# dobraczka/kiez

Hardware: AMD Instinct MI355X
Metric: source queries/sec (fit+kneighbors) + recall@k vs reference, 1/2/4/8 GPU (higher is better)
Workload: dtype f16

## Files before the change

kiez_amd/csrc/kz_common.h:

```cpp
#pragma once
#include <hip/hip_runtime.h>

#include <cstdarg>
#include <cstdint>
#include <cstdio>
#include <cstring>
#include <memory>

#include "../../include/kiez_amd.h"
#include "kz_pool_buf.h"

#define KZ_TILE 128
#define KZ_KSLICE 16
#define KZ_LIVE_MAX 1024
#define KZ_POOL_SLOTS 256

constexpr int KZ_K_LDS_PAD = 0;
constexpr int KZ_K_LONG_K = 1;
constexpr int KZ_K_FIN_WIDE = 1;
constexpr int KZ_K_RANGE_BOOT = 1;
constexpr double KZ_K_NESTED_MIN_MS = 2.0;
constexpr int KZ_K_DUAL_SHORT_DIV = 5;
constexpr int KZ_K_DUAL_SHORT_KP = 16;
constexpr int KZ_K_MIN_SPLITS = 1;
// ... 12 lines not shown
    hipStream_t stream;
    bool own_stream;
    hipEvent_t ev[12];
    int stream2_busy;
    hipStream_t stream2;
    double eps_scale;
    int force_splits;
    int chunk_rows;
    int precision;
    int dual_stride;
    int esc_bf;
    int short_ord_min_tiles;
    int short_ord;
    int dual_short_main;
    int dual_rev_long;
    int dual_short_extra;
    int dual_short_min_tiles;
    int dual_sample_short;
    int dual_overlap;
    double dual_max_gb;
    int dual_force;
    int h_q64;
    int fin_fast_div;
    double probe_min_pairs;
    int list_floor;
    int tier_probe;
    int dual_nested;
    int esc_ladder;
    int exact_rows;
    int abl;
    double floor_margin;
    int dual_rank;
    int spec_rows;
    int wide_lists;
    int wide_sel;
    void* scratch;
    size_t scratch_bytes;
    float* floor_buf;
    size_t floor_bytes;
    int* d_counters;
    int* h_counters;
    int n_cus;
    void* h_stage;
    size_t h_stage_bytes;
    int h_stage_flip;
    struct { void* ptr; size_t bytes; } pool[KZ_POOL_SLOTS];
// ... 324 lines not shown
```

kiez_amd/csrc/kz_knn.hip:

```cpp
#include <vector>

#include <algorithm>
#include <type_traits>

#include "kz_common.h"
#include "kz_bool.h"
#include "kz_floor.h"

#include "kz_knn_device.h"

template <int KP, int NRES>
__global__ __launch_bounds__(256, 3) void kz_knn_cand_kernel(KnnCandParams p) {
    extern __shared__ __attribute__((aligned(16))) char smem[];
    float* ybuf = reinterpret_cast<float*>(smem);
    const int tid = threadIdx.x;
    const int lane = tid & 63;
    const int wave = tid >> 6;
    const int j = lane & 31;
    const int h = lane >> 5;

    const int4 wd = p.work[blockIdx.x];
    const int qt = wd.x;
    const int t_begin = wd.y;
    const int t_end = wd.z;
// ... 115 lines not shown
            if (NRES == 0 || NS > NRES) {
                int sl = NRES;
                do {
                    const int sln = (sl + 1 == NS) ? NRES : sl + 1;
                    const float4 c0 = qb0, c1 = qb1;
                    slice_step(c0, c1, true, sln);
                } while (++sl < NS);
            }
            __builtin_amdgcn_sched_barrier(0);
            kz_tile_epilogue<KP>(acc, st, tile, tile == t_end - 1, h);
        }
    }
}

#include "kz_knn_bf16.h"


struct KnnFinParams {
    const float* in_key;
    const int* in_idx;
    KzListLayout lay;
    int max_m;
    int fast_div;
    int64_t q_first, q_last;
    int KP;
    int KSEL;
    int64_t list_row0;
    int64_t q_begin;
    int64_t q_count;
    const void* qraw;
    const void* yraw;
    const double* ynorm64;
    const double* qsqn;
    const double* ysqn;
    int64_t n_i;
    int d;
    int metric;
    int k;
    int exclude_self;
    const int64_t* self_ids;
    double gamma;
    const double* ystats;
    int tier_h;
    double eps_mult;
    double gamma_acc;
    const double* q_rowq;
// ... 33 lines not shown
        const int lim = min(n_sorted, k + 1);
        for (int c = 0; c < lim; ++c)
            if ((int64_t)sidx[c] == self_row) {
                self_rank = c;
                break;
            }
    }
    for (int c = lane; c < n_sorted; c += 64) {
        if (c == self_rank) continue;
        const int o = (self_rank >= 0 && c > self_rank) ? c - 1 : c;
        if (o < k) {
            od[o] = kz_output_distance<T>(sval[c], metric, p);
            oi[o] = (int64_t)sidx[c];
        }
    }
}

#ifndef KZ_FIN_ROWS_N
#define KZ_FIN_ROWS_N 1
#endif
#ifndef KZ_FIN_DEPTH
#define KZ_FIN_DEPTH 3
#endif
constexpr int KZ_FIN_ROWS = KZ_FIN_ROWS_N;
constexpr int KZ_FIN_MAXM = 4096;
constexpr int KZ_ESC_SHORT_MAX_ROWS = 2048;
constexpr int KZ_MAX_PIECES = 128;
static int kz_max_pieces(int KP, int halves) {
    const int m = KZ_FIN_MAXM / (halves * KP);
    return m < KZ_MAX_PIECES ? m : KZ_MAX_PIECES;
}

__host__ __device__ __forceinline__ int kz_fin_wave_bytes(int max_m, int KP) {
    return ((max_m * 8 + KP * 28) + 15) & ~15;
}
__host__ __device__ __forceinline__ int kz_fin_wide_wave_bytes(int max_m, int KS) {
    return ((max_m * 8 + KS * 20) + 15) & ~15;
}

template <int E>
__device__ __forceinline__ float kz_full_lists_bound(const float (&key)[E], const bool (&ok)[E], int M, int KP, int lane) {
    float bound = -INFINITY;
#pragma unroll
    for (int i = 0; i < E; ++i) {
        if (64 * i >= M) break;
        int c = ok[i] ? 1 : 0;
// ... 138 lines not shown
#pragma unroll
    for (int v = 0; v < E; ++v) {
        n_valid += __popcll(__ballot(xi[v] >= 0));
        const int lim = min(64, M - 64 * v);
        for (int jj = 0; jj < lim; ++jj) {
            const int oi = __builtin_amdgcn_readlane(xi[v], jj);
            if (oi < 0) continue;
            const float ox = __uint_as_float((unsigned)__builtin_amdgcn_readlane((int)__float_as_uint(x[v]), jj));
#pragma unroll
            for (int u = 0; u < E; ++u)
                if (64 * u < M) rank[u] += (ox > x[u] || (ox == x[u] && oi < xi[u])) ? 1 : 0;
        }
    }
#pragma unroll
    for (int u = 0; u < E; ++u) {
        if (xi[u] >= 0 && rank[u] < KP) {
            ck[rank[u]] = x[u];
            ci[rank[u]] = xi[u];
        }
    }
    return n_valid < KP ? n_valid : KP;
}

template <typename T, int FROWS, int NV = 1>
__device__ __forceinline__ void kz_finalize_query(const KnnFinParams& p, const int64_t q, const int lane, char* wbase) {
    const int KS = p.KSEL > 0 ? p.KSEL : p.KP;
    double* cv = reinterpret_cast<double*>(wbase);
    double* sv = cv + KS;
    float* ekey = reinterpret_cast<float*>(sv + KS);
    int* eidx = reinterpret_cast<int*>(ekey + p.max_m);
    float* ck = reinterpret_cast<float*>(eidx + p.max_m);
    int* ci = reinterpret_cast<int*>(ck + KS);
    int* si = ci + KS;
    const int KP = p.KP;
    const int k_eff = p.k + (p.exclude_self ? 1 : 0);
    const int64_t qrow = p.row_map ? (int64_t)p.row_map[p.q_begin + q] : p.q_begin + q;
    const int64_t qout = p.row_map ? qrow : q;
    const T* qptr = reinterpret_cast<const T*>(p.qraw) + qrow * (int64_t)p.d;
    const double qs = p.qsqn[qrow];

    const int64_t lrow = p.list_row0 + q;
    const int n_pieces = p.lay.pieces[kz_list_region(lrow, p.lay)];
    const int halves = p.lay.halves;
    const int M = n_pieces * halves * KP;
    if (p.lay.contig) {
        const int64_t l0 = kz_list_contig_off(lrow, p.lay, KP, 0);
        for (int e = lane; e < M; e += 64) {
// ... 146 lines not shown
                } else if (c < V) {
                    left_max = fmaxf(left_max, ck[c]);
                }
                cnt += (int)__popcll(mask);
            }
#pragma unroll
            for (int off = 32; off >= 1; off >>= 1) left_max = fmaxf(left_max, __shfl_xor(left_max, off, 64));
            Vr = cnt;
            ck = ekey;
            ci = eidx;
            kz_wave_sync();
        }
    } else if (V > k_eff && eps_q < INFINITY) {
        const double thr = (double)ck[k_eff - 1] * key_scale - 2.0 * eps_q;
        int cnt = 0;
        for (int c = lane; c < V; c += 64) cnt += ((double)ck[c] * key_scale >= thr) ? 1 : 0;
#pragma unroll
        for (int off = 32; off >= 1; off >>= 1) cnt += __shfl_xor(cnt, off, 64);
        Vr = cnt < k_eff ? k_eff : cnt;
    }

    const T* yraw = reinterpret_cast<const T*>(p.yraw);
    const bool vec = kz_row_vec_ok(qptr, p.d) && kz_row_vec_ok(yraw, p.d);
#ifdef KZ_NO_FIN_PIPE
    if (false) {
#else
    if (sizeof(T) == 4 && vec && p.d <= 256 * NV && Vr > 0) {
#endif
        const int k0 = 4 * lane;
        bool act[NV];
        int k0r[NV];
        double qk[4 * NV];
#pragma unroll
        for (int c = 0; c < NV; ++c) {
            act[c] = k0 + 256 * c < p.d;
            k0r[c] = act[c] ? k0 + 256 * c : 0;
            double t[4] = {0.0, 0.0, 0.0, 0.0};
            if (act[c]) {
                kz_row4(qptr, k0r[c], p.d, true, t);
                if (p.metric == KZ_COSINE) {
#pragma unroll
                    for (int e = 0; e < 4; ++e) t[e] = t[e] / qs;
                }
            }
#pragma unroll
            for (int e = 0; e < 4; ++e) qk[4 * c + e] = t[e];
// ... 171 lines not shown
            certified = V >= k_eff && (double)bound * key_scale + eps_q < exact_key(sv[k_eff - 1]);
    }
    if (Vr < V && !((double)(unsorted ? left_max : ck[Vr]) * key_scale + eps_q < exact_key(sv[k_eff - 1]))) certified = false;
    if (bound_violated) certified = false;
    if (!certified) {
        if (lane == 0) {
            const int pos = atomicAdd(p.fail_count, 1);
            p.fail_list[pos] = (int)qout;
            if (p.fail_tau) p.fail_tau[pos] = Vr >= k_eff ? sv[k_eff - 1] : (double)INFINITY;
        }
        return;
    }
    kz_emit_sorted<T>(sv, si, Vr, p.k, p.exclude_self, p.self_ids ? p.self_ids[q] : qrow, p.metric,
                      p.out_dist + qout * (int64_t)p.k, p.out_ind + qout * (int64_t)p.k, lane);
}

constexpr int KZ_FIN_QPB = 4;
#ifndef KZ_FIN_WAVES_2
#define KZ_FIN_WAVES_2 5
#endif
#ifndef KZ_FIN_WAVES
#define KZ_FIN_WAVES 7
#endif
template <typename T, int FROWS, int MINW, int NV = 1>
__global__ __launch_bounds__(256, MINW) void kz_knn_finalize_kernel(KnnFinParams p) {
    extern __shared__ __attribute__((aligned(16))) char fsm[];
    const int lane = threadIdx.x & 63;
    const int wave = __builtin_amdgcn_readfirstlane(threadIdx.x >> 6);
    char* wbase = fsm + (size_t)wave * kz_fin_wave_bytes(p.max_m, p.KSEL > 0 ? p.KSEL : p.KP);
    for (int rep = 0; rep < KZ_FIN_QPB / 4; ++rep) {
        const int64_t q = p.q_first + (int64_t)blockIdx.x * KZ_FIN_QPB + rep * 4 + wave;
        if (q >= p.q_last) break;
        kz_finalize_query<T, FROWS, NV>(p, q, lane, wbase);
        kz_wave_sync();
    }
}

#include "kz_knn_fin_wide.h"

__device__ __forceinline__ bool kz_spec_row_live(const int* __restrict__ dyn_n, int b, int cap) {
    const int n = *dyn_n;
    return n <= cap && b < n;
}

template <typename T>
__global__ __launch_bounds__(256) void kz_exact_dist_kernel(const int* __restrict__ fail_list, int batch0, int64_t q_begin,
                                                            const T* __restrict__ qraw, const T* __restrict__ yraw,
                                                            const double* __restrict__ qsqn, const double* __restrict__ ysqn,
                                                            int64_t n_i, int d, int metric, double p, double* __restrict__ vals,
                                                            const int* __restrict__ dyn_n = nullptr) {
    const int lane = threadIdx.x & 63;
    const int wave = threadIdx.x >> 6;
    const int b = blockIdx.y;
    if (dyn_n && !kz_spec_row_live(dyn_n, b, (int)gridDim.y)) return;
    const int64_t qrow = q_begin + fail_list[batch0 + b];
    for (int64_t i = (int64_t)blockIdx.x * 4 + wave; i < n_i; i += (int64_t)gridDim.x * 4) {
// ... 834 lines not shown
        while (rg + 1 < lay.n_regions && lay.pieces[rg + 1] == lay.pieces[rg]) ++rg;
        const int64_t hi = (int64_t)lay.qt_end[rg] * KZ_TILE - fp.list_row0;
        Group g = {lo < 0 ? 0 : lo, hi > q_count ? q_count : hi, lay.pieces[rg] * lay.halves * KP};
        if (g.hi > g.lo) groups[n_groups++] = g;
    }
    const hipStream_t main_stream = ctx->stream;
    const bool fork = n_groups >= 2 && ctx->stream2 && ctx->stream2 != main_stream && !ctx->stream2_busy;
    int big = 0;
    for (int g = 1; g < n_groups; ++g)
        if (groups[g].hi - groups[g].lo > groups[big].hi - groups[big].lo) big = g;
    if (fork) {
        KZ_HIP(hipEventRecord(ctx->ev[7], main_stream));
        KZ_HIP(hipStreamWaitEvent(ctx->stream2, ctx->ev[7], 0));
    }
    for (int pass = 0; pass < 2; ++pass) {
        for (int g = 0; g < n_groups; ++g) {
            const bool side = fork && g != big;
            if (fork ? (side != (pass == 0)) : pass == 1) continue;
            const hipStream_t st = side ? ctx->stream2 : main_stream;
            fp.q_first = groups[g].lo;
            fp.q_last = groups[g].hi;
            fp.max_m = groups[g].max_m;
            fp.fast_div = ctx->fin_fast_div;
            const int fin_blocks = (int)((fp.q_last - fp.q_first + KZ_FIN_QPB - 1) / KZ_FIN_QPB);
            size_t fin_lds = (size_t)4 * kz_fin_wave_bytes(fp.max_m, fp.KSEL > 0 ? fp.KSEL : KP);
            const bool wide = (fp.KSEL > 0 ? fp.KSEL : KP) > 160;
            const bool rows_vec = fp.d <= 256 && (fp.d & 3) == 0 && (((uintptr_t)fp.qraw | (uintptr_t)fp.yraw) & 15u) == 0;
            const bool wide2 = (wide || (KZ_K_FIN_WIDE >= 2 && fp.KSEL > 0)) && dtype == KZ_F32 && fp.tier_h && !fp.excl_floor && KZ_K_FIN_WIDE && rows_vec;
            const bool two_chunks = !wide && !wide2 && dtype == KZ_F32 && fp.d > 256 && fp.d <= 512 && (fp.d & 3) == 0 &&
                                    (((uintptr_t)fp.qraw | (uintptr_t)fp.yraw) & 15u) == 0;
            const void* fk = two_chunks ? (const void*)kz_knn_finalize_kernel<float, KZ_FIN_ROWS, KZ_FIN_WAVES_2, 2> : dtype == KZ_F32 ? (wide2 ? (const void*)kz_knn_finalize_wide_kernel<float, 4> : (wide ? (const void*)kz_knn_finalize_kernel<float, 8, 2> : (const void*)kz_knn_finalize_kernel<float, KZ_FIN_ROWS, KZ_FIN_WAVES>))
                                             : (wide ? (const void*)kz_knn_finalize_kernel<double, 4, 2> : (const void*)kz_knn_finalize_kernel<double, KZ_FIN_ROWS, KZ_FIN_WAVES>);
            if (wide2) fin_lds = (size_t)4 * kz_fin_wide_wave_bytes(fp.max_m, fp.KSEL);
            if (fin_lds > 65536) KZ_HIP(hipFuncSetAttribute(fk, hipFuncAttributeMaxDynamicSharedMemorySize, (int)fin_lds));
            if (wide2)
                hipLaunchKernelGGL((kz_knn_finalize_wide_kernel<float, 4>), dim3(fin_blocks), dim3(256), fin_lds, st, fp);
            else if (dtype == KZ_F32 && wide)
                hipLaunchKernelGGL((kz_knn_finalize_kernel<float, 8, 2>), dim3(fin_blocks), dim3(256), fin_lds, st, fp);
            else if (dtype == KZ_F32 && two_chunks)
                hipLaunchKernelGGL((kz_knn_finalize_kernel<float, KZ_FIN_ROWS, KZ_FIN_WAVES_2, 2>), dim3(fin_blocks), dim3(256), fin_lds, st, fp);
            else if (dtype == KZ_F32)
                hipLaunchKernelGGL((kz_knn_finalize_kernel<float, KZ_FIN_ROWS, KZ_FIN_WAVES>), dim3(fin_blocks), dim3(256), fin_lds, st, fp);
            else if (wide)
                hipLaunchKernelGGL((kz_knn_finalize_kernel<double, 4, 2>), dim3(fin_blocks), dim3(256), fin_lds, st, fp);
            else
                hipLaunchKernelGGL((kz_knn_finalize_kernel<double, KZ_FIN_ROWS, KZ_FIN_WAVES>), dim3(fin_blocks), dim3(256), fin_lds, st, fp);
        }
    }
    KZ_HIP(hipGetLastError());
    if (fork) {
        KZ_HIP(hipEventRecord(ctx->ev[11], ctx->stream2));
        KZ_HIP(hipStreamWaitEvent(main_stream, ctx->ev[11], 0));
    }
    return KZ_OK;
}

struct KzPass {
    KzListLayout lay;
    int W;
    int W0;
    float* out_key;
    int* out_idx;
    int* fail_list;
// ... 1101 lines not shown
```

kiez_amd/csrc/kz_knn_dual.h:

```cpp
#pragma once

constexpr int KZ_EVC = 1;

__global__ __launch_bounds__(256) void kz_dual_theta_kernel(const float* __restrict__ in_key, const int* __restrict__ in_idx,
                                                            KzListLayout lay, int KP, int rank, int64_t n_b, int64_t n_b_pad,
                                                            const float* __restrict__ bias_b, const double* __restrict__ a_hmax,
                                                            const double* __restrict__ b_hmax, const double* __restrict__ hscale,
                                                            float* __restrict__ theta, float* __restrict__ floor_,
                                                            const int* __restrict__ idx_to_row, int sev_cap, int* __restrict__ sev_cnt,
                                                            uint2* __restrict__ sev) {
    const int lane = threadIdx.x & 63;
    const int64_t t = (int64_t)blockIdx.x * 4 + (threadIdx.x >> 6);
    if (t >= n_b_pad) return;
    if (t >= n_b) {
        if (lane == 0) theta[t] = INFINITY;
        return;
    }
    const int M = lay.pieces[kz_list_region(t, lay)] * KP;
    const int64_t l0 = kz_list_contig_off(t, lay, KP, 0);
    float x[4];
    int valid[4];
    unsigned ux[4];
    unsigned all_or = 0u, all_and = 0xffffffffu;
    int nv = 0;
#pragma unroll
    for (int u = 0; u < 4; ++u) {
        const int e = lane + 64 * u;
        x[u] = e < M ? in_key[l0 + e] : -INFINITY;
        valid[u] = e < M && in_idx[l0 + e] >= 0;
        const unsigned b = __float_as_uint(x[u]);
        ux[u] = valid[u] ? (b ^ ((b >> 31) ? 0xffffffffu : 0x80000000u)) : 0u;
        all_or |= ux[u];
        all_and &= valid[u] ? ux[u] : 0xffffffffu;
        nv += valid[u] ? 1 : 0;
    }
#pragma unroll
// ... 28 lines not shown
            }
        }
        int base = 0;
#pragma unroll
        for (int u = 0; u < 4; ++u) {
            const bool evt = valid[u] && x[u] >= tau && tau > -INFINITY;
            const unsigned long long mask = __ballot(evt);
            if (evt) {
                const int pos = base + (int)__builtin_amdgcn_mbcnt_hi((unsigned)(mask >> 32), __builtin_amdgcn_mbcnt_lo((unsigned)mask, 0u));
                if (pos < sev_cap) sev[t * (int64_t)sev_cap + pos] = make_uint2(__float_as_uint(x[u]), (unsigned)idx_to_row[in_idx[l0 + lane + 64 * u]]);
            }
            base += (int)__popcll(mask);
        }
        if (lane == 0) sev_cnt[t] = base;
    }
    if (lane == 0) {
        const double S2 = hscale[0] * hscale[0];
        const double margin = 4.76837158203125e-07 * S2 * (a_hmax[0] * b_hmax[0] + a_hmax[2] + b_hmax[2]);
        const double th = (double)tau + (double)bias_b[t] - margin;
        float tf = (float)th;
        if ((double)tf > th) tf = nextafterf(tf, -INFINITY);
        theta[t] = tf;
        floor_[t] = tau_bound;
    }
}

__global__ __launch_bounds__(256) void kz_dual_sample_kernel(const uint4* __restrict__ packed, const float* __restrict__ bias,
                                                             int nsr, int stride, int s_tiles, int P,
                                                             uint4* __restrict__ s_packed, float* __restrict__ s_bias) {
    const int jp = blockIdx.x;
    const int n_frag = 2 * nsr * KZ_TILE;
    for (int e = threadIdx.x; e < n_frag; e += 256) {
        const int row = e & (KZ_TILE - 1), blk = e >> 7;
        const int64_t j = kz_dealt_row((int64_t)jp * KZ_TILE + row, (int64_t)s_tiles * KZ_TILE, P);
        const int64_t src_tile = (j >> 7) * stride;
        s_packed[(int64_t)jp * n_frag + e] = packed[src_tile * n_frag + blk * KZ_TILE + (j & (KZ_TILE - 1))];
        if (blk == 0) s_bias[(int64_t)jp * KZ_TILE + row] = bias[src_tile * KZ_TILE + (j & (KZ_TILE - 1))];
    }
}

__global__ void kz_dual_interleave_kernel(const int* __restrict__ perm, const float* __restrict__ theta_s, int64_t n, int64_t n_pad,
                                          int P, int* __restrict__ perm_out, float* __restrict__ theta_out) {
    const int64_t rp = (int64_t)blockIdx.x * blockDim.x + threadIdx.x;
    if (rp >= n_pad) return;
    const int64_t tiles = n_pad / KZ_TILE - 1;
    const int64_t jp = rp / KZ_TILE;
// ... 690 lines not shown
            const int KP = KPs3;
            int blocks_per_cu = 1, tpw = 1;
            KZ_DISPATCH_KP(rc, kz_h_occupancy, (n_slices, &blocks_per_cu, &tpw, KZ_K_H_WPS, KZ_K_H_WIDE, KZ_K_LDS_PAD));
            if (rc != KZ_OK) return rc;
            KzPass ps;
            rc = kz_prepare_pass(ctx, (int)s_tiles, (int)s3_tiles, kz_h_slots(n_slices, blocks_per_cu, ctx->n_cus), 256 / KP, KP, KZ_TIER_H, 0, &ps, tpw, force_s3);
            if (rc == KZ_OK) {
                KnnCandParams cp;
                memset(&cp, 0, sizeof(cp));
                cp.qpack = (const float*)q_packed.get();
                cp.ypack = (const float*)nst.s3_packed.get();
                cp.ybias = nst.s3_bias.get();
                cp.work = ps.d_work;
                cp.qt0 = 0;
                cp.n_ytiles = (int)s3_tiles;
                cp.n_qtiles = (int)s_tiles;
                cp.lay = ps.lay;
                cp.kg = b->kg;
                cp.out_key = ps.out_key;
                cp.out_idx = ps.out_idx;
                KZ_DISPATCH_KP(rc, kz_h_launch, (n_slices, ctx, cp, ps.W, KZ_K_H_WPS, KZ_K_H_WIDE));
            }
            if (rc != KZ_OK) return rc;
            hipLaunchKernelGGL(kz_dual_theta_kernel, dim3((unsigned)((s_img_rows + 3) / 4)), dim3(256), 0, ctx->stream, ps.out_key, ps.out_idx,
                               ps.lay, KP, rank3, s_img_rows, s_img_rows, q_bias.get(), ib->d_max, ia->d_max, ia->center->d_scale, nst.theta3.get(), nst.floor3.get(),
                               (const int*)nullptr, 0, (int*)nullptr, (uint2*)nullptr);
            KZ_HIP(hipGetLastError());
        }
        hipLaunchKernelGGL(kz_iota_kernel, dim3((unsigned)((s_img_rows + 255) / 256)), dim3(256), 0, ctx->stream, nst.iota3.get(), (int)s_img_rows);
        KZ_HIP(hipGetLastError());
        rc = kz_sort_pairs_f32_i32(ctx, nst.theta3.get(), nst.theta3_s.get(), nst.iota3.get(), nst.perm3.get(), (int)s_img_rows, 1);
        if (rc == KZ_OK && force_s > 1) {
            const int64_t range_rows = ((s_tiles + force_s - 1) / force_s) * KZ_TILE;
            hipLaunchKernelGGL(kz_dual_rangekey_kernel, dim3((unsigned)((s_img_rows + 255) / 256)), dim3(256), 0, ctx->stream, nst.perm3.get(), s_img_rows, range_rows,
                               nst.theta3.get(), nst.iota3.get());
            if (hipGetLastError() != hipSuccess) rc = KZ_ERR_HIP;
            if (rc == KZ_OK) rc = kz_sort_pairs_f32_i32(ctx, nst.theta3.get(), nst.floor3m.get(), nst.iota3.get(), nst.rm3.get(), (int)s_img_rows, 0);
            if (rc == KZ_OK) {
                hipLaunchKernelGGL(kz_dual_gather2_kernel, dim3((unsigned)((s_img_rows + 255) / 256)), dim3(256), 0, ctx->stream, nst.rm3.get(), nst.perm3.get(), nst.theta3_s.get(),
                                   s_img_rows, nst.iota3.get(), nst.theta3.get());
                if (hipGetLastError() != hipSuccess) rc = KZ_ERR_HIP;
                std::swap(nst.perm3, nst.iota3);
                std::swap(nst.theta3_s, nst.theta3);
            }
        }
        if (rc == KZ_OK) {
            hipLaunchKernelGGL(kz_dual_rows_of_kernel, dim3((unsigned)((s_img_rows + 255) / 256)), dim3(256), 0, ctx->stream, nst.perm3.get(), row_map.get(), s_img_rows, nst.rm3.get());
// ... 23 lines not shown
        dp2.ypack = (const float*)nst.ss_packed.get();
        dp2.ybias = nst.ss_bias.get();
        dp2.perm = nst.rm3.get();
        dp2.theta = nst.theta3_min.get();
        dp2.qnbias = nst.qnb_b.get();
        dp2.log_keys = nst.log3_keys.get();
        dp2.log_meta = nst.log3_meta.get();
        dp2.log_cnt = nst.d_cnt3.get();
        dp2.log_cap = log_cap3;
        dp2.short_pieces = force_s;
        dp2.short_kp = KPs;
        dp2.short_ksel = k;
        dp2.n_ytiles = (int)s_tiles;
        dp2.raw_lists = 1;
        dp2.max_entries = 256;
        hk2.rm3 = nst.rm3.get();
        hk2.sev_cnt = nst.sev_cnt.get();
        hk2.sev = nst.sev.get();
        dp2.post_user = &hk2;
        dp2.post_sweep = +[](void* user) -> int {
            Hook2& h = *(Hook2*)user;
            kz_ctx* ctx = h.ctx;
            const KzDualPass& d2 = *h.dp2;
            hipLaunchKernelGGL(kz_dual_theta_kernel, dim3((unsigned)((h.b_pad + 3) / 4)), dim3(256), 0, ctx->stream, d2.lists_key, d2.lists_idx,
                               d2.lists_lay, d2.lists_KP, h.rank, h.b_n, h.b_pad, h.ib->bias, h.ia->d_max, h.ib->d_max, h.ib->center->d_scale,
                               h.theta, h.floor_, h.rm3, h.sev_cap, h.sev_cnt, h.sev);
            KZ_HIP(hipGetLastError());
            return kz_dual_enqueue_chain(*h.rv3);
        };
        kz_knn_stats st2;
        ctx->stream2_busy = 1;
        rc = kz_knn_impl(ctx, b, 0, b->n, a, k, 0, nullptr, KzResearch(), d_dist_ba, d_ind_ba, &st2, &dp2);
        if (rc != KZ_OK) return rc;
        if (dp2.broken || !dp2.post_called) {
            then = 1;
            return KZ_OK;
        }
        nested_sweep_ms = st2.main_kernel_ms;
    } else {
        hipLaunchKernelGGL(kz_dual_sample_kernel, dim3((unsigned)s_tiles), dim3(256), 0, ctx->stream, (const uint4*)ia->packed, ia->bias,
                           n_slices, stride, (int)s_tiles, force_s > 0 ? force_s : 1, (uint4*)s_packed.get(), s_bias.get());
        KZ_HIP(hipGetLastError());
        const int KP = KPs;
        int blocks_per_cu = 1, tpw = 1;
        KZ_DISPATCH_KP(rc, kz_h_occupancy, (n_slices, &blocks_per_cu, &tpw, KZ_K_H_WPS, KZ_K_H_WIDE, KZ_K_LDS_PAD));
        if (rc != KZ_OK) return rc;
        KzPass ps;
        rc = kz_prepare_pass(ctx, (int)b_tiles, (int)s_tiles, kz_h_slots(n_slices, blocks_per_cu, ctx->n_cus), 256 / KP, KP, KZ_TIER_H, 0, &ps, tpw, force_s);
        if (rc != KZ_OK) return rc;
        KnnCandParams cp;
        memset(&cp, 0, sizeof(cp));
        cp.qpack = (const float*)ib->packed;
        cp.ypack = (const float*)s_packed.get();
        cp.ybias = s_bias.get();
        cp.work = ps.d_work;
        cp.qt0 = 0;
        cp.n_ytiles = (int)s_tiles;
        cp.n_qtiles = (int)b_tiles;
        cp.lay = ps.lay;
        cp.kg = b->kg;
        cp.out_key = ps.out_key;
        cp.out_idx = ps.out_idx;
        KZ_DISPATCH_KP(rc, kz_h_launch, (n_slices, ctx, cp, ps.W, KZ_K_H_WPS, KZ_K_H_WIDE));
        if (rc != KZ_OK) return rc;
        hipLaunchKernelGGL(kz_dual_theta_kernel, dim3((unsigned)((b_pad + 3) / 4)), dim3(256), 0, ctx->stream, ps.out_key, ps.out_idx,
                           ps.lay, KP, rank, b->n, b_pad, ib->bias, ia->d_max, ib->d_max, ib->center->d_scale, theta.get(), floor_.get(),
                           (const int*)nullptr, 0, (int*)nullptr, (uint2*)nullptr);
        KZ_HIP(hipGetLastError());
    }
    hipLaunchKernelGGL(kz_iota_kernel, dim3((unsigned)((b_pad + 255) / 256)), dim3(256), 0, ctx->stream, iota.get(), (int)b_pad);
    hipLaunchKernelGGL(kz_dual_fill_kernel, dim3((unsigned)((b_pad + 255) / 256)), dim3(256), 0, ctx->stream, theta_s.get(), b_pad, INFINITY);
    KZ_HIP(hipGetLastError());
    rc = kz_sort_pairs_f32_i32(ctx, theta.get(), theta_s.get(), iota.get(), perm.get(), (int)b->n, 1);
    if (rc != KZ_OK) return rc;
    int main_pieces = 0;
    if (ctx->dual_short_main && KP > 16) {
        const int per = KZ_K_DUAL_SHORT_DIV * (KZ_K_DUAL_SHORT_KP / 16);
        const int P = (k + per - 1) / per;
        if (P >= 2 && P * KZ_K_DUAL_SHORT_KP <= 512 && KP > KZ_K_DUAL_SHORT_KP && b_tiles - 1 >= (int64_t)ctx->dual_short_min_tiles * P) main_pieces = P;
    }
    if (main_pieces > 0) {
        hipLaunchKernelGGL(kz_dual_interleave_kernel, dim3((unsigned)((b_pad + 255) / 256)), dim3(256), 0, ctx->stream, perm.get(), theta_s.get(), b->n,
                           b_pad, main_pieces, iota.get(), theta.get());
        KZ_HIP(hipGetLastError());
        std::swap(perm, iota);
        std::swap(theta_s, theta);
    }
    hipLaunchKernelGGL(kz_dual_tilemin_kernel, dim3((unsigned)((b_pad + 255) / 256)), dim3(256), 0, ctx->stream, theta_s.get(), b->n, b_pad, theta_min.get());
// ... 155 lines not shown
```

kiez_amd/csrc/kz_options.h:

```cpp
#pragma once
#include <cstddef>

#include "kz_common.h"

enum { KZ_OPT_INT = 0, KZ_OPT_BOOL = 1, KZ_OPT_F64 = 2 };
enum { KZ_OPT_PUBLIC = 1, KZ_OPT_SET = 2  };

struct KzOption {
    const char* name;
    int kind;
    size_t offset;
    double lo, hi;
    double dflt;
    unsigned flags;
    double allowed[4];
    int n_allowed;
    const char* doc;
};

#define KZ_O(field) offsetof(kz_ctx, field)
static const KzOption KZ_OPTIONS[] = {
    {"precision", KZ_OPT_INT, KZ_O(precision), 0, 2, 0, KZ_OPT_PUBLIC, {}, 0,
     "first-pass operands: 0 fp16 on centred operands (default), 2 split-bf16, 1 float32; the neighbour order is the float64 one either way"},
    {"dual_stride", KZ_OPT_INT, KZ_O(dual_stride), 0, 64, 1, KZ_OPT_PUBLIC, {}, 0,
     "kz_knn_dual: every n-th tile of a is in the threshold sample; 1 = chosen from the shapes, 0 = always two ordinary searches"},
    {"dual_max_gb", KZ_OPT_F64, KZ_O(dual_max_gb), 0, 1e6, 0, KZ_OPT_PUBLIC, {}, 0,
     "kz_knn_dual: transient footprint it may claim, GiB (0 = 32); beyond it, or beyond what the device has free, it searches twice"},
    {"eps_scale", KZ_OPT_F64, KZ_O(eps_scale), 1e-300, 1e300, 1.0, KZ_OPT_PUBLIC, {}, 0,
     "multiplies the certification bound (test knob: a huge value sends every row to the exact float64 kernels)"},
    {"force_splits", KZ_OPT_INT, KZ_O(force_splits), 0, 64, 0, 0, {}, 0, "fixed index split count (0 = automatic)"},
    {"chunk_rows", KZ_OPT_INT, KZ_O(chunk_rows), 0, 1e9, 0, 0, {}, 0, "query rows per chunk (0 = by list length)"},
    {"h_q64", KZ_OPT_INT, KZ_O(h_q64), 0, 2, 2, 0, {}, 0, "64-queries-per-wave build: 2 where it pays, 1 wherever built, 0 never"},
    {"short_ord", KZ_OPT_BOOL, KZ_O(short_ord), 0, 1, 1, 0, {}, 0, "ordinary search: k / 5 lists of 16 on a row-dealt image (13 .. 320 neighbours)"},
    {"short_ord_min_tiles", KZ_OPT_INT, KZ_O(short_ord_min_tiles), 1, 1e9, 48, 0, {}, 0, "... when an index range has at least this many tiles"},
    {"esc_bf", KZ_OPT_BOOL, KZ_O(esc_bf), 0, 1, 1, 0, {}, 0, "split-bf16 operands before the float32 ones for rows the fp16 tier cannot certify"},
    {"tier_probe", KZ_OPT_INT, KZ_O(tier_probe), 0, 65536, 1024, 0, {}, 0, "rows of the strided sample a large search sends through the fp16 pass first (0 = off)"},
    {"probe_min_pairs", KZ_OPT_F64, KZ_O(probe_min_pairs), 0, 1e300, 5e10, 0, {}, 0, "searches of fewer distance pairs take neither the tier probe nor a floor"},
    {"esc_ladder", KZ_OPT_BOOL, KZ_O(esc_ladder), 0, 1, 1, 0, {}, 0, "a pass without a probe that leaves more than half of its rows uncertified tries the wide route on a sample of them before the split-bf16 tier"},
    {"exact_rows", KZ_OPT_INT, KZ_O(exact_rows), 0, 3, 3, 0, {}, 0, "exact float64 distance kernels: 0 one pair per wave, 1 + many pairs per wave step (float32 rows of d <= 512), 2 + one pair per LANE for batches of >= 32 rows (kz_exact_lanes.h), 3 (default) + the RANGE re-search for >= 128 rows (kz_range.h: only the index rows within the rounding bound of a row's k-th candidate); all bit-identical"},
    {"abl", KZ_OPT_INT, KZ_O(abl), 0, 31, 0, 0, {}, 0, "diagnostics, bit mask: 1 = an ordinary one-range fp16 sweep runs twice, the second (timed) one from the first one's final thresholds; 2 = with a -DKZ_ABL_STAMP build and KZ_STAMP_FILE set, clock stamps of every workgroup of an ordinary fp16 sweep; 4 = the range re-search's log holds 4096 groups (overflow path); 8 = the range re-search treats every row as one without k candidates (hand-back path); 16 = no grouped ranges (one range per row)"},
    {"spec_rows", KZ_OPT_INT, KZ_O(spec_rows), 0, 64, 64, 0, {}, 0, "exact kernels launched speculatively behind every finalize for at most this many uncertified rows (0 = off)"},
    {"wide_lists", KZ_OPT_INT, KZ_O(wide_lists), 2, 32, 32, KZ_OPT_SET, {0}, -1, "fp16 tier's wide route: lists of 16 per query (0 = off)"},
    {"wide_sel", KZ_OPT_INT, KZ_O(wide_sel), 16, 512, 256, 0, {}, 0, "... entries of those lists the finalize kernel selects"},
    {"floor_margin", KZ_OPT_F64, KZ_O(floor_margin), 0, 1e6, 1.3, 0, {}, 0, "seeded lists: the largest shortfall of the probe below the model, times this (0: the model itself -- half of the rows are searched again; test knob)"},
    {"dual_rank", KZ_OPT_INT, KZ_O(dual_rank), -1, 128, 0, 0, {}, 0, "rank of the sample key that becomes a row's event threshold (0 automatic, -1 = k + 1; 1: many rows short of events, test knob)"},
    {"list_floor", KZ_OPT_INT, KZ_O(list_floor), 0, 1, 1, 0, {}, 0, "seeded candidate lists (population floor from a probe)"},
    {"fin_fast_div", KZ_OPT_INT, KZ_O(fin_fast_div), 0, 1, 1, 0, {}, 0, "cosine re-rank through one reciprocal per candidate row (bit-identical)"},
    {"dual_force", KZ_OPT_BOOL, KZ_O(dual_force), 0, 1, 0, 0, {}, 0, "run the shared sweep also where its cost model says it does not pay (tests)"},
    {"dual_overlap", KZ_OPT_BOOL, KZ_O(dual_overlap), 0, 1, 1, 0, {}, 0, "reverse direction's chain on the second stream"},
    {"dual_nested", KZ_OPT_BOOL, KZ_O(dual_nested), 0, 1, 1, 0, {}, 0, "sampled rows are swept by the sample sweep only (itself a shared sweep)"},
    {"dual_rev_long", KZ_OPT_BOOL, KZ_O(dual_rev_long), 0, 1, 1, 0, {}, 0, "reverse lists of twice the list length"},
    {"dual_sample_short", KZ_OPT_BOOL, KZ_O(dual_sample_short), 0, 1, 1, 0, {}, 0, "sample sweep keeps lists of 16 (32) over several ranges"},
    {"dual_short_main", KZ_OPT_BOOL, KZ_O(dual_short_main), 0, 1, 1, 0, {}, 0, "main sweep keeps k / dual_short_div lists of 16 (13 .. 110 neighbours)"},
    {"dual_short_extra", KZ_OPT_INT, KZ_O(dual_short_extra), 1, 200, 48, 0, {}, 0, "entries selected beyond k on that route"},
    {"dual_short_min_tiles", KZ_OPT_INT, KZ_O(dual_short_min_tiles), 1, 1e9, 128, 0, {}, 0, "... taken when an index range has at least this many tiles"},
};
#undef KZ_O
static const int KZ_N_OPTIONS = (int)(sizeof(KZ_OPTIONS) / sizeof(KZ_OPTIONS[0]));

static inline void kz_option_store(kz_ctx* c, const KzOption& o, double v) {
    char* p = reinterpret_cast<char*>(c) + o.offset;
    if (o.kind == KZ_OPT_F64)
        *reinterpret_cast<double*>(p) = v;
    else
        *reinterpret_cast<int*>(p) = o.kind == KZ_OPT_BOOL ? (v != 0 ? 1 : 0) : (int)v;
}
static inline void kz_options_defaults(kz_ctx* c) {
    for (int i = 0; i < KZ_N_OPTIONS; ++i) kz_option_store(c, KZ_OPTIONS[i], KZ_OPTIONS[i].dflt);
}
```

Measured before the change: 2.737 million.

## Re-rank two candidates per wave in finalize and batch dual theta rows

Adds a pair-mode float32 finalize path. Each half-wave re-ranks one candidate row of d <= 256, so two candidates are processed per wave step, with software-pipelined loads and a 32-lane reduction; it is enabled by default through a new option. The dual theta kernel now handles four rows per wave, packing short lists (<=16 or <=32 entries) into lane groups and ranking them with DPP row rotations instead of one row per wave. Both changes aim to cut idle lanes and latency stalls in small-row work. The finalize change only applies to f32 inputs, and the workload is f16, so it may not run here; the theta change applies only to the dual route.

```diff
diff --git a/kiez_amd/csrc/kz_common.h b/kiez_amd/csrc/kz_common.h
--- a/kiez_amd/csrc/kz_common.h
+++ b/kiez_amd/csrc/kz_common.h
@@ -58,6 +58,7 @@
     int dual_force;
     int h_q64;
     int fin_fast_div;
+    int fin_pairs;
     double probe_min_pairs;
     int list_floor;
     int tier_probe;
diff --git a/kiez_amd/csrc/kz_knn.hip b/kiez_amd/csrc/kz_knn.hip
--- a/kiez_amd/csrc/kz_knn.hip
+++ b/kiez_amd/csrc/kz_knn.hip
@@ -161,6 +161,7 @@
     KzListLayout lay;
     int max_m;
     int fast_div;
+    int pairs;
     int64_t q_first, q_last;
     int KP;
     int KSEL;
@@ -240,6 +241,12 @@
 #ifndef KZ_FIN_DEPTH
 #define KZ_FIN_DEPTH 3
 #endif
+#ifndef KZ_FIN_WAVES_PAIRS
+#define KZ_FIN_WAVES_PAIRS 6
+#endif
+#ifndef KZ_FIN_PAIR_DEPTH
+#define KZ_FIN_PAIR_DEPTH 2
+#endif
 constexpr int KZ_FIN_ROWS = KZ_FIN_ROWS_N;
 constexpr int KZ_FIN_MAXM = 4096;
 constexpr int KZ_ESC_SHORT_MAX_ROWS = 2048;
@@ -424,7 +431,7 @@
     return n_valid < KP ? n_valid : KP;
 }
 
-template <typename T, int FROWS, int NV = 1>
+template <typename T, int FROWS, int NV = 1, bool PAIRS = false>
 __device__ __forceinline__ void kz_finalize_query(const KnnFinParams& p, const int64_t q, const int lane, char* wbase) {
     const int KS = p.KSEL > 0 ? p.KSEL : p.KP;
     double* cv = reinterpret_cast<double*>(wbase);
@@ -617,6 +624,111 @@
 
     const T* yraw = reinterpret_cast<const T*>(p.yraw);
     const bool vec = kz_row_vec_ok(qptr, p.d) && kz_row_vec_ok(yraw, p.d);
+#if !defined(KZ_NO_FIN_PIPE)
+    static_assert(!PAIRS || (sizeof(T) == 4 && FROWS == 1 && NV == 1), "the pair layout is that of float32 rows of up to 256 elements");
+    if (PAIRS && vec && p.d <= 256 && Vr > 0) {
+        const int half = lane >> 5;
+        bool act[2];
+        int k0r[2];
+        double qk[8];
+#pragma unroll
+        for (int c = 0; c < 2; ++c) {
+            const int k0 = 4 * (lane & 31) + 128 * c;
+            act[c] = k0 < p.d;
+            k0r[c] = act[c] ? k0 : 0;
+            double t[4] = {0.0, 0.0, 0.0, 0.0};
+            if (act[c]) {
+                kz_row4(qptr, k0r[c], p.d, true, t);
+                if (p.metric == KZ_COSINE) {
+#pragma unroll
+                    for (int e = 0; e < 4; ++e) t[e] = t[e] / qs;
+                }
+            }
+#pragma unroll
+            for (int e = 0; e < 4; ++e) qk[4 * c + e] = t[e];
+        }
+        auto issue = [&](int c0, float4 (&buf)[2], double& ysb) {
+            const int yi = ci[min(c0 + half, Vr - 1)];
+            ysb = p.ysqn[yi];
+            const float* row = reinterpret_cast<const float*>(yraw) + (int64_t)yi * p.d;
+#pragma unroll
+            for (int c = 0; c < 2; ++c) buf[c] = *reinterpret_cast<const float4*>(row + k0r[c]);
+        };
+        auto reduce = [&](int c0, const float4 (&buf)[2], const double ysb) {
+            double a[2] = {0.0, 0.0};
+            bool done = false;
+            if (p.metric == KZ_COSINE && p.fast_div) {
+                const double rcp = 1.0 / ysb;
+                const bool inf = ((int)((unsigned long long)__double_as_longlong(rcp) >> 32) & 0x7ff00000) == 0x7ff00000;
+                if (__ballot(inf) == 0ull) {
+#pragma unroll
+                    for (int c = 0; c < 2; ++c) {
+                        const double yk[4] = {(double)buf[c].x, (double)buf[c].y, (double)buf[c].z, (double)buf[c].w};
+                        if (act[c]) {
+#pragma unroll
+                            for (int e = 0; e < 4; ++e) a[c] = fma(qk[4 * c + e], kz_div_shared(yk[e], ysb, rcp), a[c]);
+                        }
+                    }
+                    done = true;
+                }
+            }
+            if (!done) {
+#pragma unroll
+                for (int c = 0; c < 2; ++c) {
+                    const double yk[4] = {(double)buf[c].x, (double)buf[c].y, (double)buf[c].z, (double)buf[c].w};
+                    if (act[c]) {
+                        if (p.metric == KZ_COSINE) {
+#pragma unroll
+                            for (int e = 0; e < 4; ++e) a[c] = fma(qk[4 * c + e], yk[e] / ysb, a[c]);
+                        } else {
+#pragma unroll
+                            for (int e = 0; e < 4; ++e) a[c] = fma(qk[4 * c + e], yk[e], a[c]);
+                        }
+                    }
+                }
+            }
+            double dot = a[0] + a[1];
+#pragma unroll
+            for (int off = 16; off >= 1; off >>= 1) dot += __shfl_xor(dot, off, 64);
+            double v;
+            if (p.metric == KZ_COSINE) {
+                v = fmin(fmax(1.0 - dot, 0.0), 2.0);
+            } else {
+                v = fmax((qs + ysb) - 2.0 * dot, 0.0);
+            }
+            if ((lane & 31) == 0 && c0 + half < Vr) cv[c0 + half] = v;
+        };
+#if KZ_FIN_PAIR_DEPTH == 2
+        float4 b0[2], b1[2];
+        double y0, y1;
+        issue(0, b0, y0);
+        for (int c0 = 0;;) {
+            issue(c0 + 2, b1, y1);
+            reduce(c0, b0, y0);
+            if ((c0 += 2) >= Vr) break;
+            issue(c0 + 2, b0, y0);
+            reduce(c0, b1, y1);
+            if ((c0 += 2) >= Vr) break;
+        }
+#else
+        float4 b0[2], b1[2], b2[2];
+        double y0, y1, y2;
+        issue(0, b0, y0);
+        issue(2, b1, y1);
+        for (int c0 = 0;;) {
+            issue(c0 + 4, b2, y2);
+            reduce(c0, b0, y0);
+            if ((c0 += 2) >= Vr) break;
+            issue(c0 + 4, b0, y0);
+            reduce(c0, b1, y1);
+            if ((c0 += 2) >= Vr) break;
+            issue(c0 + 4, b1, y1);
+            reduce(c0, b2, y2);
+            if ((c0 += 2) >= Vr) break;
+        }
+#endif
+    } else
+#endif
 #ifdef KZ_NO_FIN_PIPE
     if (false) {
 #else
@@ -834,7 +946,7 @@
 #ifndef KZ_FIN_WAVES
 #define KZ_FIN_WAVES 7
 #endif
-template <typename T, int FROWS, int MINW, int NV = 1>
+template <typename T, int FROWS, int MINW, int NV = 1, bool PAIRS = false>
 __global__ __launch_bounds__(256, MINW) void kz_knn_finalize_kernel(KnnFinParams p) {
     extern __shared__ __attribute__((aligned(16))) char fsm[];
     const int lane = threadIdx.x & 63;
@@ -843,7 +955,7 @@
     for (int rep = 0; rep < KZ_FIN_QPB / 4; ++rep) {
         const int64_t q = p.q_first + (int64_t)blockIdx.x * KZ_FIN_QPB + rep * 4 + wave;
         if (q >= p.q_last) break;
-        kz_finalize_query<T, FROWS, NV>(p, q, lane, wbase);
+        kz_finalize_query<T, FROWS, NV, PAIRS>(p, q, lane, wbase);
         kz_wave_sync();
     }
 }
@@ -1724,6 +1836,7 @@
             fp.q_last = groups[g].hi;
             fp.max_m = groups[g].max_m;
             fp.fast_div = ctx->fin_fast_div;
+            fp.pairs = ctx->fin_pairs && dtype == KZ_F32;
             const int fin_blocks = (int)((fp.q_last - fp.q_first + KZ_FIN_QPB - 1) / KZ_FIN_QPB);
             size_t fin_lds = (size_t)4 * kz_fin_wave_bytes(fp.max_m, fp.KSEL > 0 ? fp.KSEL : KP);
             const bool wide = (fp.KSEL > 0 ? fp.KSEL : KP) > 160;
@@ -1731,7 +1844,8 @@
             const bool wide2 = (wide || (KZ_K_FIN_WIDE >= 2 && fp.KSEL > 0)) && dtype == KZ_F32 && fp.tier_h && !fp.excl_floor && KZ_K_FIN_WIDE && rows_vec;
             const bool two_chunks = !wide && !wide2 && dtype == KZ_F32 && fp.d > 256 && fp.d <= 512 && (fp.d & 3) == 0 &&
                                     (((uintptr_t)fp.qraw | (uintptr_t)fp.yraw) & 15u) == 0;
-            const void* fk = two_chunks ? (const void*)kz_knn_finalize_kernel<float, KZ_FIN_ROWS, KZ_FIN_WAVES_2, 2> : dtype == KZ_F32 ? (wide2 ? (const void*)kz_knn_finalize_wide_kernel<float, 4> : (wide ? (const void*)kz_knn_finalize_kernel<float, 8, 2> : (const void*)kz_knn_finalize_kernel<float, KZ_FIN_ROWS, KZ_FIN_WAVES>))
+            const bool pairs = fp.pairs && !wide && !wide2 && !two_chunks && rows_vec;
+            const void* fk = two_chunks ? (const void*)kz_knn_finalize_kernel<float, KZ_FIN_ROWS, KZ_FIN_WAVES_2, 2> : dtype == KZ_F32 ? (wide2 ? (const void*)kz_knn_finalize_wide_kernel<float, 4> : (wide ? (const void*)kz_knn_finalize_kernel<float, 8, 2> : pairs ? (const void*)kz_knn_finalize_kernel<float, 1, KZ_FIN_WAVES_PAIRS, 1, true> : (const void*)kz_knn_finalize_kernel<float, KZ_FIN_ROWS, KZ_FIN_WAVES>))
                                              : (wide ? (const void*)kz_knn_finalize_kernel<double, 4, 2> : (const void*)kz_knn_finalize_kernel<double, KZ_FIN_ROWS, KZ_FIN_WAVES>);
             if (wide2) fin_lds = (size_t)4 * kz_fin_wide_wave_bytes(fp.max_m, fp.KSEL);
             if (fin_lds > 65536) KZ_HIP(hipFuncSetAttribute(fk, hipFuncAttributeMaxDynamicSharedMemorySize, (int)fin_lds));
@@ -1741,6 +1855,8 @@
                 hipLaunchKernelGGL((kz_knn_finalize_kernel<float, 8, 2>), dim3(fin_blocks), dim3(256), fin_lds, st, fp);
             else if (dtype == KZ_F32 && two_chunks)
                 hipLaunchKernelGGL((kz_knn_finalize_kernel<float, KZ_FIN_ROWS, KZ_FIN_WAVES_2, 2>), dim3(fin_blocks), dim3(256), fin_lds, st, fp);
+            else if (dtype == KZ_F32 && pairs)
+                hipLaunchKernelGGL((kz_knn_finalize_kernel<float, 1, KZ_FIN_WAVES_PAIRS, 1, true>), dim3(fin_blocks), dim3(256), fin_lds, st, fp);
             else if (dtype == KZ_F32)
                 hipLaunchKernelGGL((kz_knn_finalize_kernel<float, KZ_FIN_ROWS, KZ_FIN_WAVES>), dim3(fin_blocks), dim3(256), fin_lds, st, fp);
             else if (wide)
diff --git a/kiez_amd/csrc/kz_knn_dual.h b/kiez_amd/csrc/kz_knn_dual.h
--- a/kiez_amd/csrc/kz_knn_dual.h
+++ b/kiez_amd/csrc/kz_knn_dual.h
@@ -2,16 +2,13 @@
 
 constexpr int KZ_EVC = 1;
 
-__global__ __launch_bounds__(256) void kz_dual_theta_kernel(const float* __restrict__ in_key, const int* __restrict__ in_idx,
-                                                            KzListLayout lay, int KP, int rank, int64_t n_b, int64_t n_b_pad,
-                                                            const float* __restrict__ bias_b, const double* __restrict__ a_hmax,
-                                                            const double* __restrict__ b_hmax, const double* __restrict__ hscale,
-                                                            float* __restrict__ theta, float* __restrict__ floor_,
-                                                            const int* __restrict__ idx_to_row, int sev_cap, int* __restrict__ sev_cnt,
-                                                            uint2* __restrict__ sev) {
-    const int lane = threadIdx.x & 63;
-    const int64_t t = (int64_t)blockIdx.x * 4 + (threadIdx.x >> 6);
-    if (t >= n_b_pad) return;
+__device__ __forceinline__ void kz_dual_theta_row(const float* __restrict__ in_key, const int* __restrict__ in_idx,
+                                                  const KzListLayout& lay, int KP, int rank, const int64_t t, int64_t n_b,
+                                                  const float* __restrict__ bias_b, const double* __restrict__ a_hmax,
+                                                  const double* __restrict__ b_hmax, const double* __restrict__ hscale,
+                                                  float* __restrict__ theta, float* __restrict__ floor_,
+                                                  const int* __restrict__ idx_to_row, int sev_cap, int* __restrict__ sev_cnt,
+                                                  uint2* __restrict__ sev, const int lane) {
     if (t >= n_b) {
         if (lane == 0) theta[t] = INFINITY;
         return;
@@ -86,6 +83,115 @@
         if ((double)tf > th) tf = nextafterf(tf, -INFINITY);
         theta[t] = tf;
         floor_[t] = tau_bound;
+    }
+}
+
+#define KZ_ROW_ROR(v, n) ((unsigned)__builtin_amdgcn_update_dpp(0, (int)(v), 0x120 + (n), 0xf, 0xf, false))
+#define KZ_THETA_COUNT(o_)       \
+    {                            \
+        const unsigned o = (o_); \
+        gt += o > ux ? 1 : 0;    \
+        ge += o >= ux ? 1 : 0;   \
+    }
+#define KZ_THETA_COUNT_ROR(src)                                                                                  \
+    KZ_THETA_COUNT(KZ_ROW_ROR(src, 1)) KZ_THETA_COUNT(KZ_ROW_ROR(src, 2)) KZ_THETA_COUNT(KZ_ROW_ROR(src, 3))    \
+    KZ_THETA_COUNT(KZ_ROW_ROR(src, 4)) KZ_THETA_COUNT(KZ_ROW_ROR(src, 5)) KZ_THETA_COUNT(KZ_ROW_ROR(src, 6))    \
+    KZ_THETA_COUNT(KZ_ROW_ROR(src, 7)) KZ_THETA_COUNT(KZ_ROW_ROR(src, 8)) KZ_THETA_COUNT(KZ_ROW_ROR(src, 9))    \
+    KZ_THETA_COUNT(KZ_ROW_ROR(src, 10)) KZ_THETA_COUNT(KZ_ROW_ROR(src, 11)) KZ_THETA_COUNT(KZ_ROW_ROR(src, 12)) \
+    KZ_THETA_COUNT(KZ_ROW_ROR(src, 13)) KZ_THETA_COUNT(KZ_ROW_ROR(src, 14)) KZ_THETA_COUNT(KZ_ROW_ROR(src, 15))
+template <int LG>
+__device__ __forceinline__ void kz_dual_theta_rows(const float* __restrict__ in_key, const int* __restrict__ in_idx,
+                                                   const KzListLayout& lay, int KP, int M, int rank, const int64_t tw, int64_t n_b,
+                                                   int64_t n_b_pad, const float* __restrict__ bias_b, const double* __restrict__ a_hmax,
+                                                   const double* __restrict__ b_hmax, const double* __restrict__ hscale,
+                                                   float* __restrict__ theta, float* __restrict__ floor_,
+                                                   const int* __restrict__ idx_to_row, int sev_cap, int* __restrict__ sev_cnt,
+                                                   uint2* __restrict__ sev, const int lane) {
+    const int g = lane / LG, e = lane & (LG - 1);
+    const int64_t t = tw + g;
+    const bool row = t < n_b;
+    const bool in = row && e < M;
+    const int64_t l0 = kz_list_contig_off(tw, lay, KP, 0) + (int64_t)g * M;
+    const float x = in ? in_key[l0 + e] : -INFINITY;
+    const int xi = in ? in_idx[l0 + e] : -1;
+    const bool valid = xi >= 0;
+    const unsigned b = __float_as_uint(x);
+    const unsigned ux = valid ? (b ^ ((b >> 31) ? 0xffffffffu : 0x80000000u)) : 0u;
+    int gt = 0, ge = 1;
+    KZ_THETA_COUNT_ROR(ux)
+    if (LG == 32) {
+        const unsigned px = (unsigned)__shfl_xor((int)ux, 16, 64);
+        KZ_THETA_COUNT(px)
+        KZ_THETA_COUNT_ROR(px)
+    }
+    unsigned thr = valid && gt < rank && rank <= ge ? ux : 0u;
+#pragma unroll
+    for (int off = LG >> 1; off >= 1; off >>= 1) thr = max(thr, (unsigned)__shfl_xor((int)thr, off, 64));
+    const float tau = thr ? __uint_as_float(thr ^ ((thr >> 31) ? 0x80000000u : 0xffffffffu)) : -INFINITY;
+    float tau_bound = tau;
+    if (sev_cnt) {
+        int c = valid ? 1 : 0;
+        float mn = valid ? x : INFINITY;
+        for (int off = KP >> 1; off >= 1; off >>= 1) {
+            c += __shfl_xor(c, off, 64);
+            mn = fminf(mn, __shfl_xor(mn, off, 64));
+        }
+        float bound = c == KP && e < M ? mn : -INFINITY;
+#pragma unroll
+        for (int off = LG >> 1; off >= 1; off >>= 1) bound = fmaxf(bound, __shfl_xor(bound, off, 64));
+        tau_bound = fmaxf(tau_bound, bound);
+        const bool evt = valid && x >= tau && tau > -INFINITY;
+        const unsigned long long gmask = (LG == 32 ? 0xffffffffull : 0xffffull) << (g * LG);
+        const unsigned long long mask = __ballot(evt) & gmask;
+        if (evt) {
+            const int pos = (int)__builtin_amdgcn_mbcnt_hi((unsigned)(mask >> 32), __builtin_amdgcn_mbcnt_lo((unsigned)mask, 0u));
+            if (pos < sev_cap) sev[t * (int64_t)sev_cap + pos] = make_uint2(__float_as_uint(x), (unsigned)idx_to_row[xi]);
+        }
+        if (e == 0 && row) sev_cnt[t] = (int)__popcll(mask);
+    }
+    if (e == 0 && row) {
+        const double S2 = hscale[0] * hscale[0];
+        const double margin = 4.76837158203125e-07 * S2 * (a_hmax[0] * b_hmax[0] + a_hmax[2] + b_hmax[2]);
+        const double th = (double)tau + (double)bias_b[t] - margin;
+        float tf = (float)th;
+        if ((double)tf > th) tf = nextafterf(tf, -INFINITY);
+        theta[t] = tf;
+        floor_[t] = tau_bound;
+    } else if (e == 0 && t < n_b_pad) {
+        theta[t] = INFINITY;
+    }
+}
+#undef KZ_THETA_COUNT_ROR
+#undef KZ_THETA_COUNT
+#undef KZ_ROW_ROR
+
+constexpr int KZ_THETA_WROWS = 4;
+__global__ __launch_bounds__(256) void kz_dual_theta_kernel(const float* __restrict__ in_key, const int* __restrict__ in_idx,
+                                                            KzListLayout lay, int KP, int rank, int64_t n_b, int64_t n_b_pad,
+                                                            const float* __restrict__ bias_b, const double* __restrict__ a_hmax,
+                                                            const double* __restrict__ b_hmax, const double* __restrict__ hscale,
+                                                            float* __restrict__ theta, float* __restrict__ floor_,
+                                                            const int* __restrict__ idx_to_row, int sev_cap, int* __restrict__ sev_cnt,
+                                                            uint2* __restrict__ sev) {
+    const int lane = threadIdx.x & 63;
+    const int64_t t0 = ((int64_t)blockIdx.x * 4 + __builtin_amdgcn_readfirstlane(threadIdx.x >> 6)) * KZ_THETA_WROWS;
+    if (t0 >= n_b_pad) return;
+    if (t0 >= n_b) {
+        if (lane < KZ_THETA_WROWS && t0 + lane < n_b_pad) theta[t0 + lane] = INFINITY;
+        return;
+    }
+    const int M = lay.pieces[kz_list_region(t0, lay)] * KP;
+    if (M <= 16) {
+        kz_dual_theta_rows<16>(in_key, in_idx, lay, KP, M, rank, t0, n_b, n_b_pad, bias_b, a_hmax, b_hmax, hscale, theta, floor_, idx_to_row,
+                               sev_cap, sev_cnt, sev, lane);
+    } else if (M <= 32) {
+        for (int r = 0; r < KZ_THETA_WROWS; r += 2)
+            kz_dual_theta_rows<32>(in_key, in_idx, lay, KP, M, rank, t0 + r, n_b, n_b_pad, bias_b, a_hmax, b_hmax, hscale, theta, floor_,
+                                   idx_to_row, sev_cap, sev_cnt, sev, lane);
+    } else {
+        for (int r = 0; r < KZ_THETA_WROWS && t0 + r < n_b_pad; ++r)
+            kz_dual_theta_row(in_key, in_idx, lay, KP, rank, t0 + r, n_b, bias_b, a_hmax, b_hmax, hscale, theta, floor_, idx_to_row, sev_cap,
+                              sev_cnt, sev, lane);
     }
 }
 
@@ -822,7 +928,7 @@
                 KZ_DISPATCH_KP(rc, kz_h_launch, (n_slices, ctx, cp, ps.W, KZ_K_H_WPS, KZ_K_H_WIDE));
             }
             if (rc != KZ_OK) return rc;
-            hipLaunchKernelGGL(kz_dual_theta_kernel, dim3((unsigned)((s_img_rows + 3) / 4)), dim3(256), 0, ctx->stream, ps.out_key, ps.out_idx,
+            hipLaunchKernelGGL(kz_dual_theta_kernel, dim3((unsigned)((s_img_rows + 4 * KZ_THETA_WROWS - 1) / (4 * KZ_THETA_WROWS))), dim3(256), 0, ctx->stream, ps.out_key, ps.out_idx,
                                ps.lay, KP, rank3, s_img_rows, s_img_rows, q_bias.get(), ib->d_max, ia->d_max, ia->center->d_scale, nst.theta3.get(), nst.floor3.get(),
                                (const int*)nullptr, 0, (int*)nullptr, (uint2*)nullptr);
             KZ_HIP(hipGetLastError());
@@ -892,7 +998,7 @@
             Hook2& h = *(Hook2*)user;
             kz_ctx* ctx = h.ctx;
             const KzDualPass& d2 = *h.dp2;
-            hipLaunchKernelGGL(kz_dual_theta_kernel, dim3((unsigned)((h.b_pad + 3) / 4)), dim3(256), 0, ctx->stream, d2.lists_key, d2.lists_idx,
+            hipLaunchKernelGGL(kz_dual_theta_kernel, dim3((unsigned)((h.b_pad + 4 * KZ_THETA_WROWS - 1) / (4 * KZ_THETA_WROWS))), dim3(256), 0, ctx->stream, d2.lists_key, d2.lists_idx,
                                d2.lists_lay, d2.lists_KP, h.rank, h.b_n, h.b_pad, h.ib->bias, h.ia->d_max, h.ib->d_max, h.ib->center->d_scale,
                                h.theta, h.floor_, h.rm3, h.sev_cap, h.sev_cnt, h.sev);
             KZ_HIP(hipGetLastError());
@@ -933,7 +1039,7 @@
         cp.out_idx = ps.out_idx;
         KZ_DISPATCH_KP(rc, kz_h_launch, (n_slices, ctx, cp, ps.W, KZ_K_H_WPS, KZ_K_H_WIDE));
         if (rc != KZ_OK) return rc;
-        hipLaunchKernelGGL(kz_dual_theta_kernel, dim3((unsigned)((b_pad + 3) / 4)), dim3(256), 0, ctx->stream, ps.out_key, ps.out_idx,
+        hipLaunchKernelGGL(kz_dual_theta_kernel, dim3((unsigned)((b_pad + 4 * KZ_THETA_WROWS - 1) / (4 * KZ_THETA_WROWS))), dim3(256), 0, ctx->stream, ps.out_key, ps.out_idx,
                            ps.lay, KP, rank, b->n, b_pad, ib->bias, ia->d_max, ib->d_max, ib->center->d_scale, theta.get(), floor_.get(),
                            (const int*)nullptr, 0, (int*)nullptr, (uint2*)nullptr);
         KZ_HIP(hipGetLastError());
diff --git a/kiez_amd/csrc/kz_options.h b/kiez_amd/csrc/kz_options.h
--- a/kiez_amd/csrc/kz_options.h
+++ b/kiez_amd/csrc/kz_options.h
@@ -46,6 +46,7 @@
     {"dual_rank", KZ_OPT_INT, KZ_O(dual_rank), -1, 128, 0, 0, {}, 0, "rank of the sample key that becomes a row's event threshold (0 automatic, -1 = k + 1; 1: many rows short of events, test knob)"},
     {"list_floor", KZ_OPT_INT, KZ_O(list_floor), 0, 1, 1, 0, {}, 0, "seeded candidate lists (population floor from a probe)"},
     {"fin_fast_div", KZ_OPT_INT, KZ_O(fin_fast_div), 0, 1, 1, 0, {}, 0, "cosine re-rank through one reciprocal per candidate row (bit-identical)"},
+    {"fin_pairs", KZ_OPT_BOOL, KZ_O(fin_pairs), 0, 1, 1, 0, {}, 0, "pipelined re-rank of float32 rows of d <= 256: two candidate rows per wave step, one per lane half (bit-identical)"},
     {"dual_force", KZ_OPT_BOOL, KZ_O(dual_force), 0, 1, 0, 0, {}, 0, "run the shared sweep also where its cost model says it does not pay (tests)"},
     {"dual_overlap", KZ_OPT_BOOL, KZ_O(dual_overlap), 0, 1, 1, 0, {}, 0, "reverse direction's chain on the second stream"},
     {"dual_nested", KZ_OPT_BOOL, KZ_O(dual_nested), 0, 1, 1, 0, {}, 0, "sampled rows are swept by the sample sweep only (itself a shared sweep)"},
```

Result: slower. 2.674 million (-2.3%).
